# dselivanov/rsparse

Hardware: AMD Instinct MI355X
Metric: als_iterations_per_sec (higher is better)
Workload: dtype f32 (Gram products of rows > 512 / <= 32 non-zeros as 2 x fp16 / 3 x bf16 split terms of the fp32 operands, fp32 accumulate; everything else fp32); 1 GPU; WRMF implicit ALS, CG(3), synthetic 10000000x1000000, 500155883 nnz, rank 128, lambda 0.1; survey_config=3, feedback=implicit, n_items=1000000, nnz=500155883, rank=128, solver=conjugate_gradient, cg_steps=3, parallelism=rows sharded x1, factors replicated

## Files before the change

### rsparse_amd/build.py

```python
import subprocess
import sys
import time
from concurrent.futures import ThreadPoolExecutor
from pathlib import Path

PKG = Path(__file__).resolve().parent
CSRC = PKG / "csrc"
SRC = [CSRC / n for n in ("wrmf_kernels.hip", "wrmf_cgq.hip", "wrmf_cgp.hip", "wrmf_ne.hip", "wrmf_chol.hip", "wrmf_chol_wave.hip", "wrmf_chol_mf.hip", "wrmf_cg_mf.hip", "wrmf_chol_lr.hip",
                          "wrmf_topk.hip", "wrmf_topk_large.hip", "wrmf_similar.hip", "wrmf_metrics.hip", "wrmf_hits.hip", "wrmf_lists.hip", "wrmf_diversity.hip", "wrmf_mmr.hip", "wrmf_ranks.hip", "wrmf_score.hip", "wrmf_softals.hip", "wrmf_itemknn.hip", "wrmf_candidates.hip", "wrmf_sample.hip", "wrmf_sample_weighted.hip", "wrmf_split.hip", "wrmf_confidence.hip", "wrmf_events.hip", "wrmf_explain.hip", "wrmf_init.hip", "wrmf_ingest.hip", "wrmf_nnls.hip", "wrmf_bias.hip", "wrmf_lu.hip",
                          "wrmf_f64.hip", "wrmf_wide.hip", "wrmf_wide_cg.hip", "wrmf_ctx_kernels.hip", "wrmf_schedule.cpp", "wrmf_capi.cpp", "wrmf_f64_capi.cpp", "wrmf_capi_host.cpp", "wrmf_ctx.cpp")]
HEADERS = [CSRC / "wrmf_chol_mf.attrs.csv", CSRC / "wrmf_mf.h", CSRC / "wrmf_internal.h", CSRC / "wrmf_capi_common.h", CSRC / "wrmf_schedule.h", CSRC / "wrmf_device.h", CSRC / "wrmf_sample_team.h", CSRC / "wrmf_wave.h", CSRC / "wrmf_csr_rows.h", CSRC / "wrmf_ldlt.h", CSRC / "wrmf_f64.h", PKG.parent / "include" / "rsparse_wrmf_hip.h"]
DEPS = SRC + HEADERS
OUT = PKG / "lib" / "librsparse_wrmf_hip.so"
FLAGS = ["--offload-arch=gfx950", "-O3", "-std=c++17", "-fPIC"]


EXTRA_FLAGS = {n: ["-mllvm", "-forceattrs-csv-path=" + str(CSRC / "wrmf_chol_mf.attrs.csv"), "-fno-slp-vectorize"] for n in ("wrmf_chol_mf.hip", "wrmf_cg_mf.hip")}
AUDITED = {"wrmf_chol_mf.hip", "wrmf_cg_mf.hip"}
REG_LIMIT = {"wrmf_cg_mf.hip": 512}
NO_SPILL = {"wrmf_cgq.hip": ("14als_cgq_kernelILi128ELi24ELi4ELi4E",),
            "wrmf_cgp.hip": ("14als_cgp_kernelILb0ELb1ELi16ELb1E",),
            "wrmf_explain.hip": ("14explain_kernelIfLi128E",),
            "wrmf_sample.hip": ("13sample_kernelILi64E", "13sample_kernelILi256E"),
            "wrmf_sample_weighted.hip": ("22sample_weighted_kernelILi64E", "22sample_weighted_kernelILi256E"),
            "wrmf_hits.hip": ("18hit_metrics_kernelILb0E", "18hit_metrics_kernelILb1E"),
            "wrmf_lists.hip": ("19list_metrics_kernelILb0E", "19list_metrics_kernelILb1E"),
            "wrmf_diversity.hip": ("21list_diversity_kernelI", "21item_inv_norms_kernelI"),
            "wrmf_mmr.hip": ("10mmr_kernelI",),
            "wrmf_confidence.hip": ("conf_moments_kernel", "conf_moments_finish_kernel", "conf_table_kernel", "conf_apply_kernel"),
            "wrmf_events.hip": ("events_pack_kernel", "events_now_kernel", "events_heads_kernel", "events_reduce_kernel",
                                "events_long_chunks_kernel", "events_long_finish_kernel"),
            "wrmf_cg_mf.hip": ("rsparse_hip_als_cg_mf_implicit", "rsparse_hip_als_cg_mf_implicit_any"),
            "wrmf_softals.hip": ("softals_span_kernel", "softals_finish_kernel", "softals_empty_rows_kernel"),
            "wrmf_itemknn.hip": ("knn_scatter_kernel", "knn_mask_kernel", "knn_select_kernel"),
            "wrmf_split.hip": ("split_count_wave_kernel", "split_count_team_kernel", "split_write_wave_kernel", "split_write_team_kernel")}
RESOURCE_FLAG = "-Rpass-analysis=kernel-resource-usage"


def resource_violations(remarks, patterns, limit=256):
    import re
    rows, cur = [], None
    for line in remarks.splitlines():
        m = re.search(r"remark:\s+(.*?) \[-Rpass", line)
# ... 103 lines not shown
```

### rsparse_amd/csrc/wrmf_capi.cpp

```cpp
#include "../../include/rsparse_wrmf_hip.h"

#include <cxxabi.h>

#include <algorithm>
#include <cfloat>
#include <cmath>
#include <cstdlib>
#include <cstring>
#include <string>
#include <vector>

#include "wrmf_capi_common.h"

using namespace rsparse_hip;

struct rsparse_hip_csc {
  DevCSC d;
  int device = 0;
  std::vector<void*> owned;
};

namespace {
thread_local std::string g_err;
}
// ... 115 lines not shown
  if (int rc = upload(m, cut.segs, &L.segs)) return rc;
  if (int rc = upload(m, cut.split_rows, &L.split_rows)) return rc;
  return upload(m, cut.split_ptr, &L.split_ptr);
}
int upload_deal(rsparse_hip_csc& m, const NeDeal& deal, NeListSet& L) {
  L.wg = deal.wg();
  if (int rc = upload(m, deal.rows, &L.rows)) return rc;
  return upload(m, deal.ptr, &L.ptr);
}

int build_schedule(rsparse_hip_csc& m, const int32_t* host_col_ptrs) {
  DevCSC& d = m.d;
  int cus = 256;
  HIP_TRY(hipDeviceGetAttribute(&cus, hipDeviceAttributeMultiprocessorCount, m.device));
  d.q_cfg = cgq_default_cfg();
  SchedulePlan plan;
  if (!plan_schedule(host_col_ptrs, d.n_cols, cus, [](int len) { return cgq_bucket_of(len, cgq_default_cfg()); }, plan))
    return fail(RSPARSE_HIP_ERR_INVALID, "col_ptrs is not non-decreasing");
  d.max_len = plan.max_len; d.nnz_long = plan.nnz_long; d.n_empty = plan.n_empty;
  d.short_max = kTileNnz; d.n_long = plan.n_long;
  for (int b = 0; b < 7; b++) d.q_off[b] = plan.off[b];
  for (int b = 0; b < 6; b++) d.q_nnz[b] = plan.nnz[b];
  d.q_pair_first = plan.pair_first; d.q_team4_first = plan.team4_first;
  d.q_team4_wide_first = plan.team4_wide_first;
  d.q_gt32 = plan.gt32; d.q_gt48 = plan.gt48; d.q_lr_first = plan.lr_first; d.q_n_lr = plan.n_lr;
  d.q_n_chol_long = plan.n_chol_long; d.q_n_nec = plan.n_nec;
  int rc;
  if ((rc = upload(m, plan.order, &d.q_order))) return rc;
  if ((rc = upload(m, plan.stream_off, &d.q_stream_off))) return rc;
  if ((rc = upload_cut(m, plan.cut, d.q_ne))) return rc;
  d.q_ne1 = d.q_ne;
  if ((rc = upload_deal(m, plan.fine, d.q_ne))) return rc;
  if ((rc = upload_deal(m, plan.coarse, d.q_ne1))) return rc;
  if (plan.nec_is_ne) {
    d.q_nec = d.q_ne;
  } else {
    if ((rc = upload_cut(m, plan.cut_nec, d.q_nec))) return rc;
    if ((rc = upload_deal(m, plan.nec, d.q_nec))) return rc;
  }
  return RSPARSE_HIP_OK;
}

bool use_cgq(int rank, const void* X, const void* Y) {
  return rank % 4 == 0 && ((reinterpret_cast<uintptr_t>(X) | reinterpret_cast<uintptr_t>(Y)) & 15) == 0;
}

int check_common(int n_rows, int n_cols, const void* col_ptrs, const void* X, const void* Y, int rank) {
// ... 105 lines not shown
    a.rhs_vals = bias ? bias->rhs_vals : nullptr;
    a.loss_tgt = bias ? bias->loss_tgt : nullptr;
    a.rhs_init = bias ? bias->rhs_init : nullptr;
    a.loss_tgt_const = bias ? bias->tgt_const : 1.f;
    a.gbias = (solver == RSPARSE_SOLVER_CONJUGATE_GRADIENT && implicit && bias) ? bias->gbias : 0.f;
    const bool wave_cg = wide_cg_wave_supported(a, solver) && (d.q_order || d.max_len <= kWideCgMaxLen);
    hipError_t we = wave_cg ? launch_wide_cg_wave(a, implicit, kWideCgMaxLen, d.max_len > kWideCgMaxLen ? d.q_order : nullptr, 0, s)
                            : launch_als_wide(a, implicit, solver, g_ws.wide_m2, g_ws.wide_lu, s);
    if (we != hipSuccess) return hip_fail(we, wave_cg ? "launch_wide_cg_wave" : "launch_als_wide");
    if ((we = launch_sum_partials(g_ws.partials, wave_cg ? (size_t)grid_w : (size_t)grid, outw, s, g_ws.partials + g_ws.partial_slots())) != hipSuccess)
      return hip_fail(we, "launch_sum_partials");
    return RSPARSE_HIP_OK;
  }
  const bool cg = solver == RSPARSE_SOLVER_CONJUGATE_GRADIENT;
  const bool cgq = cg && use_cgq(rank, d_X, d_Y);
  QSchedule qs;
  qs.order = d.q_order;
  qs.cfg = d.q_cfg;
  qs.pair_first = d.q_pair_first;
  for (int b = 0; b < 7; b++) qs.off[b] = d.q_off[b];
  qs.team4_first = (implicit && bias && bias->gbias != 0.f) ? d.q_off[2] : d.q_team4_first;
  qs.team4_wide_first = (implicit && bias && bias->gbias != 0.f) ? d.q_off[2] : d.q_team4_wide_first;
  qs.pair_wide = cgp_wide_supported(rank, implicit, implicit && bias && bias->gbias != 0.f);
  qs.pair_quad = cgp_quad_supported(rank, implicit, implicit && bias && bias->gbias != 0.f);
  const bool cg_mf = cgq && implicit && !bias && cg_mf_supported(rank, implicit) && d.q_order && d.q_off[1] > d.q_n_nec;
  if (cg_mf) {
    qs.mf_rows = d.q_order + d.q_n_nec;
    qs.mf_n = d.q_off[1] - d.q_n_nec;
  }
  const bool chol_mf = chol_mf_supported(rank) && !cg && solver == RSPARSE_SOLVER_CHOLESKY && !bias && d.q_order && ne_supported(rank) &&
                       use_cgq(rank, d_X, d_Y) && d.q_lr_first > d.q_off[1];
  const int mf_first = d.q_off[1];
  const int n_mf = chol_mf ? d.q_lr_first - mf_first : 0;
  const bool nec_lists = padded_rank(rank) > 64 && d.q_nec.wg > 0 && !chol_mf;
  const bool ne_chol = !cg && solver == RSPARSE_SOLVER_CHOLESKY && !bias && (nec_lists || d.q_ne.wg > 0 || chol_mf) &&
                       ne_supported(rank) && use_cgq(rank, d_X, d_Y);
  qs.ne = (cg_mf || (ne_chol && nec_lists)) ? d.q_nec : ((implicit && padded_rank(rank) == 128) ? d.q_ne : d.q_ne1);
  const size_t chol_base = chol2_loss_slots(d.n_cols);
  const size_t slots = cgq ? cgq_loss_slots(qs, rank, implicit) : (cg ? cg_loss_slots(d.n_cols, d.n_long)
                                   : (solver == RSPARSE_SOLVER_NNLS ? chol_loss_slots(d.n_cols)
                                      : chol_base + (ne_chol ? (size_t)(qs.ne.entries + qs.ne.nsplit) : 0) +
                                            (size_t)(chol_mf ? chol_mf_loss_slots(n_mf, implicit) : 0) + (size_t)kLuGrid));
  if ((rc = g_ws.ensure_partials(slots))) return rc;
  double* out = d_loss_rows_out ? d_loss_rows_out : g_ws.scalars;
  if (d.n_cols == 0) {
    HIP_TRY(hipMemsetAsync(out, 0, sizeof(double), s));
// ... 1307 lines not shown
```

### rsparse_amd/csrc/wrmf_cgq.hip

```cpp
#include <algorithm>

#include "wrmf_internal.h"
#include "wrmf_device.h"

namespace rsparse_hip {
namespace {

using namespace dev;

constexpr int kGvFirstMinCapq = 16;
constexpr int kStreamPrefixQ = 4;
constexpr int kIdxPrefetchMaxWpr = 2;

constexpr int kMaxSavedSweeps = 4;

template <int KP>
struct QG {
  static constexpr int RPN = KP / 16;
  static constexpr int VW = RPN >= 4 ? 4 : RPN;
  static constexpr int NV = RPN / VW;
  __device__ static __forceinline__ int elem(int i, int r) { return (r / VW) * (16 * VW) + i * VW + (r % VW); }
};

template <int VW>
struct Piece;
template <>
struct Piece<4> { using type = float4; };
template <>
struct Piece<2> { using type = float2; };

__device__ __forceinline__ float groups_reduce_scatter4(const float a0, const float a1, const float a2, const float a3) {
  const auto s01 = __builtin_amdgcn_permlane16_swap(__float_as_uint(a0), __float_as_uint(a1), false, false);
  const float c = __uint_as_float(s01[0]) + __uint_as_float(s01[1]);
  const auto s23 = __builtin_amdgcn_permlane16_swap(__float_as_uint(a2), __float_as_uint(a3), false, false);
  const float d = __uint_as_float(s23[0]) + __uint_as_float(s23[1]);
  const auto t = __builtin_amdgcn_permlane32_swap(__float_as_uint(c), __float_as_uint(d), false, false);
  return __uint_as_float(t[0]) + __uint_as_float(t[1]);
}
template <int KP, int CAPQ, int WAVES, int WPR, int STREAM, bool IMPLICIT, int DMF = 0>
struct QSmem {
  static constexpr size_t gram_floats = (IMPLICIT && DMF != 1) ? (size_t)KP * KP : 0;
  static constexpr size_t vec_floats = IMPLICIT ? (size_t)WAVES * KP : 0;
  static constexpr size_t red_floats = WPR > 1 ? (size_t)2 * WAVES * KP + 2 * WAVES : 0;
  static constexpr bool cv_lds = !STREAM && CAPQ * (KP / 16) > 128;
  static constexpr bool wideq = !STREAM && CAPQ * (KP / 16) > 160;
  static constexpr size_t tsv_floats = (STREAM && !IMPLICIT) ? 0 : (size_t)WAVES * (cv_lds ? 3 : 2) * CAPQ * 4;
  static constexpr size_t pre_floats = STREAM ? (size_t)WAVES * kStreamPrefixQ * 4 * KP : 0;
  static constexpr int dmf_ps = KP + 8, dmf_os = KP + 4;
  static constexpr size_t dmf_floats = DMF ? (size_t)WAVES * dmf_ps + (size_t)WAVES * dmf_os : 0;
  static constexpr size_t pfx_floats =
      (!STREAM && WPR > kIdxPrefetchMaxWpr && (CAPQ == 16 || CAPQ == 20 || CAPQ == 24)) ? (size_t)WAVES * 2 * CAPQ * 4 : 0;
  static constexpr size_t wl_floats = cv_lds ? (size_t)WAVES * 2 : 0;
  static constexpr size_t xs_floats = cv_lds ? (size_t)WAVES * KP : 0;
  static constexpr size_t bytes =
      (gram_floats + vec_floats + red_floats + tsv_floats + pre_floats + dmf_floats + pfx_floats + wl_floats + xs_floats) * 4 + 16;
};

template <int KP, int CAPQ, int WAVES, int WPR, int STREAM, bool IMPLICIT, int DMF = 0, bool GB = false, bool KFULL = false>
__global__ __launch_bounds__(WAVES * 64, 2) void als_cgq_kernel(AlsArgs a, const int32_t* __restrict__ rows, int n_rows,
                                                             int rows_per_team, size_t loss_slot0) {
  using G_ = QG<KP>;
  constexpr int RPN = G_::RPN, VW = G_::VW, NV = G_::NV, CAP = CAPQ * 4, TEAMS = WAVES / WPR;
  using piece_t = typename Piece<VW>::type;
  using SM = QSmem<KP, CAPQ, WAVES, WPR, STREAM, IMPLICIT, DMF>;
  static_assert(WAVES % WPR == 0, "teams must tile the workgroup");
  constexpr bool GRS = RPN == 8 && VW == 4;
  auto groups_all_reduce8 = [](float(&a8)[RPN]) {
    if constexpr (RPN == 8) {
      const float r0 = groups_reduce_scatter4(a8[0], a8[1], a8[2], a8[3]);
      const float r1 = groups_reduce_scatter4(a8[4], a8[5], a8[6], a8[7]);
      float g0[4], g1[4];
      rows_to_all<4>(r0, g0);
      rows_to_all<4>(r1, g1);
#pragma unroll
      for (int e = 0; e < 4; e++) a8[e] = g0[e], a8[4 + e] = g1[e];
    }
  };
  static_assert(!DMF || (IMPLICIT && KP == 128 && WAVES == 4 && WPR == 1 && STREAM == 0), "DMF geometry");
  static_assert(DMF != 1 || CAPQ == 8, "register-resident G terms: only the 8-quad kernel has the 64 registers");
  static_assert(!GB || IMPLICIT, "the global bias of explicit feedback is removed from the data (R/model_WRMF.R:278-282)");
  const float gbias = GB ? a.gbias : 0.f, ltgt = GB ? a.loss_tgt_const : 1.f;
  extern __shared__ __attribute__((aligned(16))) char smem[];
  float* sG = reinterpret_cast<float*>(smem);
  float* sVec = sG + SM::gram_floats;
  float* sRed = sVec + SM::vec_floats;
  float* sRedL = sRed + (WPR > 1 ? 2 * WAVES * KP : 0);
  float* sTsv = sVec + SM::vec_floats + SM::red_floats;
  float* sPre = sTsv + SM::tsv_floats;
  float* sPfx = sPre + SM::pre_floats;
  _Float16* sPh = reinterpret_cast<_Float16*>(sPre + SM::pre_floats);
  _Float16* sPl = sPh + WAVES * SM::dmf_ps;
  float* sOut = reinterpret_cast<float*>(sPl + WAVES * SM::dmf_ps);

  const int tid = threadIdx.x, lane = tid & 63, wv = rfl(tid >> 6);
  const int g = lane >> 4, i = lane & 15;
  const int team = wv / WPR, tw = wv % WPR;
  const int k = KFULL ? KP : a.k;
  if constexpr (IMPLICIT && DMF == 0) {
    constexpr int GU = (KP * KP) % (8 * WAVES * 64) == 0 ? 8 : ((KP * KP) % (2 * WAVES * 64) == 0 ? 2 : 1);
    static_assert((KP * KP) % (GU * WAVES * 64) == 0, "the Gramian copy walks whole batches");
    for (int e0 = tid; e0 < KP * KP; e0 += GU * WAVES * 64) {
      float gv[GU];
#pragma unroll
      for (int u = 0; u < GU; u++) {
        const int e = e0 + u * WAVES * 64, r = e / KP, c = e % KP;
        gv[u] = a.XtX[(size_t)min(r, k - 1) * k + min(c, k - 1)];
      }
#pragma unroll
      for (int u = 0; u < GU; u++) {
        const int e = e0 + u * WAVES * 64, r = e / KP, c = e % KP;
        sG[e] = (r < k && c < k) ? gv[u] : 0.f;
      }
// ... 76 lines not shown
  const int team_global = blockIdx.x * TEAMS + team;
  const int total_teams = gridDim.x * TEAMS;

  auto row_index = [&](int itn) { return team_global + itn * total_teams; };
  int row_c = 0, p1_c = 0, p2_c = 0, row_n = 0;
  if (rows_per_team > 0 && row_index(0) < n_rows) {
    row_c = rows[row_index(0)];
    p1_c = a.col_ptrs[row_c];
    p2_c = a.col_ptrs[row_c + 1];
  }
  if (rows_per_team > 1 && row_index(1) < n_rows) row_n = rows[row_index(1)];
  for (int it = 0; it < rows_per_team; ++it) {
    const int ri = row_index(it);
    const bool have = ri < n_rows;
    if (WPR == 1 && !DMF && !have) break;
    const int row = have ? rfl(row_c) : 0;
    const int p1 = have ? rfl(p1_c) : 0;
    const int p2 = have ? rfl(p2_c) : 0;
    constexpr bool META_LATE = WIDEQ && !KFULL;
#define RSP_ADVANCE_META()                                                      \
    {                                                                           \
      int p1_n = 0, p2_n = 0, row_nn = 0;                                       \
      if (it + 1 < rows_per_team && row_index(it + 1) < n_rows) {               \
        p1_n = a.col_ptrs[row_n];                                               \
        p2_n = a.col_ptrs[row_n + 1];                                           \
      }                                                                         \
      if (it + 2 < rows_per_team && row_index(it + 2) < n_rows) row_nn = rows[row_index(it + 2)]; \
      row_c = row_n;                                                            \
      p1_c = p1_n;                                                              \
      p2_c = p2_n;                                                              \
      row_n = row_nn;                                                           \
    }
    if constexpr (!META_LATE) RSP_ADVANCE_META()
    const int cnt = p2 - p1;
    float* yrow = a.Y + (size_t)row * k;
    if (!GB && WPR == 1 && cnt <= 0) {
      if (!DMF || have)
        for (int e = lane; e < k; e += 64) yrow[e] = 0.f;
      if constexpr (!DMF) continue;
    }
    constexpr int PQ = STREAM ? kStreamPrefixQ : 0, PCAP = PQ * 4, PTEAM = PCAP * WPR;
    const int pre = STREAM ? min(cnt, PTEAM) : 0;
    const int pw = STREAM ? max(0, min(PCAP, pre - tw * PCAP)) : 0;
    const int nchunks = (cnt - pre + CAP - 1) / CAP;
    constexpr bool resident = STREAM == 0;
    const float lam_use =
        IMPLICIT ? 0.f : (float)(a.lambda_loss * (a.dynamic_lambda ? (double)(float)cnt : 1.0));

// ... 256 lines not shown
      float lacc = 0.f;
      float vinv = 0.f;
      if constexpr (DMF) {
        if (mode != 2) {
          float vmax = 0.f;
#pragma unroll
          for (int rr = 0; rr < RPN; rr++) vmax = fmaxf(vmax, fabsf(v[rr]));
          vmax = row16_max(vmax);
          const int ve = fp16_scale_exp(vmax);
          const float vs = __uint_as_float((unsigned)ve << 23);
          vinv = __uint_as_float((unsigned)(254 - ve) << 23) * (mode == 0 ? -1.f : 1.f);
          if (g < NV) {
            float w4[VW];
#pragma unroll
            for (int c = 0; c < VW; c++) w4[c] = (g == 0 ? v[c] : v[VW + c]) * vs;
            unsigned h0, l0, h1, l1;
            split_f16(w4[0], w4[1], h0, l0);
            split_f16(w4[2], w4[3], h1, l1);
            const int off = wv * SM::dmf_ps + g * 16 * VW + i * VW;
            *reinterpret_cast<uint2*>(sPh + off) = make_uint2(h0, h1);
            *reinterpret_cast<uint2*>(sPl + off) = make_uint2(l0, l1);
          }
          __syncthreads();
          f32x4 d0[2], d1[2];
#pragma unroll
          for (int t = 0; t < 2; t++) d0[t] = d1[t] = f32x4{0.f, 0.f, 0.f, 0.f};
          const int nb = (lane & 3) * SM::dmf_ps + 8 * (lane >> 4);
#pragma unroll
          for (int ks = 0; ks < 4; ks++) {
            const f16x8 bh = *reinterpret_cast<const f16x8*>(sPh + nb + 32 * ks);
            const f16x8 bl = *reinterpret_cast<const f16x8*>(sPl + nb + 32 * ks);
#pragma unroll
            for (int t = 0; t < 2; t++) {
              f16x8 ah, al;
              if constexpr (DMF == 1) {
                ah = gAh[t][ks];
                al = gAl[t][ks];
              } else {
                ah = *reinterpret_cast<const f16x8*>(sGf + ((t * 4 + ks) * 2 + 0) * 1024 + lane * 16);
                al = *reinterpret_cast<const f16x8*>(sGf + ((t * 4 + ks) * 2 + 1) * 1024 + lane * 16);
              }
              d0[t] = __builtin_amdgcn_mfma_f32_16x16x32_f16(ah, bh, d0[t], 0, 0, 0);
              d1[t] = __builtin_amdgcn_mfma_f32_16x16x32_f16(ah, bl, d1[t], 0, 0, 0);
              d1[t] = __builtin_amdgcn_mfma_f32_16x16x32_f16(al, bh, d1[t], 0, 0, 0);
            }
          }
          if ((lane & 15) < 4) {
#pragma unroll
            for (int t = 0; t < 2; t++) {
              const f32x4 d = (d0[t] + d1[t]) * ginv;
              *reinterpret_cast<f32x4*>(sOut + (lane & 15) * SM::dmf_os + 32 * wv + 16 * t + 4 * (lane >> 4)) = d;
            }
          }
        }
      }
      if (live) {
        if constexpr (IMPLICIT && !DMF) {
          if (mode != 2) {
            wave_sync();
            if (g == 0) {
#pragma unroll
              for (int b = 0; b < NV; b++) {
                piece_t pc;
                float* pf = reinterpret_cast<float*>(&pc);
#pragma unroll
                for (int c = 0; c < VW; c++) pf[c] = v[b * VW + c];
                *reinterpret_cast<piece_t*>(vec + b * 16 * VW + i * VW) = pc;
              }
            }
            wave_sync();
          }
        }
        auto dense_part = [&]() {
          if (IMPLICIT && !DMF && mode != 2) {
            const float sign = mode == 0 ? -1.f : 1.f;
// ... 330 lines not shown
    }
  }
  if (lane == 0) a.loss_partials[loss_slot0 + (size_t)blockIdx.x * WAVES + wv] = CVLDS ? *wl_lds : wloss;
}

struct BucketDef { int waves, wpr, capq, stream, max_len; };
constexpr int kNB = 6;
constexpr int kNCfg = 2;
constexpr BucketDef kBuckets[kNCfg][kNB] = {
    {{8, 8, 16, 1, 0x7fffffff}, {8, 8, 16, 0, 512}, {4, 4, 16, 0, 256}, {4, 2, 16, 0, 128}, {4, 1, 16, 0, 64}, {4, 1, 8, 0, 32}},
    {{8, 8, 16, 1, 0x7fffffff}, {4, 4, 32, 0, 512}, {4, 2, 32, 0, 256}, {4, 1, 32, 0, 128}, {4, 1, 16, 0, 64}, {4, 1, 8, 0, 32}},
};
constexpr int cfg_of_kp(int KP) { return KP == 64 ? 1 : 0; }
constexpr int kTeam4Waves = 4, kTeam4Capq = 20;
static_assert(kTeam4Max == kTeam4Waves * kTeam4Capq * 4, "wrmf_internal.h's split and the kernel's capacity");
constexpr int kTeam4WideCapq = 24;
static_assert(kTeam4WideMax == kTeam4Waves * kTeam4WideCapq * 4, "wrmf_schedule.h's split and the wide kernel's capacity");
static_assert(kTeam4Max < kTeam4WideMax && kTeam4WideMax < 512, "the 4-wave launches take bucket 1's rows from its short end");
static_assert(QSmem<128, kTeam4WideCapq, kTeam4Waves, kTeam4Waves, 0, true>::bytes <= 80 * 1024, "the wide team kernel's LDS");
constexpr bool team4_split(int KP, bool GB) { return KP == 128 && !GB; }
int team4_first(const QSchedule& q) { return std::min(std::max(q.team4_first, q.off[1]), q.off[2]); }
int team4_wide_first(const QSchedule& q) { return std::min(std::max(q.team4_wide_first, q.off[1]), team4_first(q)); }

template <int KP, int WAVES, int CAPQ, int WPR, int STREAM, bool IMPLICIT, bool GB, int DMF = 0, bool KFULL = false>
hipError_t launch_bucket(const AlsArgs& a, const int32_t* rows, int n_rows, int grid, size_t slot0, hipStream_t s,
                         hipEvent_t* ev_slot) {
  if (n_rows <= 0) return hipSuccess;
  constexpr bool kDmfGeometry = IMPLICIT && KP == 128 && WAVES == 4 && WPR == 1 && (CAPQ == 8 || CAPQ == 16) && STREAM == 0;
  if constexpr (kDmfGeometry && !DMF) {
    return launch_bucket<KP, WAVES, CAPQ, WPR, STREAM, IMPLICIT, GB, CAPQ == 8 ? 1 : 2>(a, rows, n_rows, grid, slot0, s, ev_slot);
  } else {
    if constexpr (!KFULL && STREAM == 0 && !(DMF == 1 && !GB)) {
      if (a.k == KP)
        return launch_bucket<KP, WAVES, CAPQ, WPR, STREAM, IMPLICIT, GB, DMF, true>(a, rows, n_rows, grid, slot0, s, ev_slot);
    }
    constexpr int TEAMS = WAVES / WPR;
    auto kern = als_cgq_kernel<KP, CAPQ, WAVES, WPR, STREAM, IMPLICIT, DMF, GB, KFULL>;
    const size_t lds = QSmem<KP, CAPQ, WAVES, WPR, STREAM, IMPLICIT, DMF>::bytes;
    hipError_t err = hipFuncSetAttribute(reinterpret_cast<const void*>(kern),
                                         hipFuncAttributeMaxDynamicSharedMemorySize, (int)lds);
    if (err != hipSuccess) return err;
    const int total_teams = grid * TEAMS;
    const int rpt = (n_rows + total_teams - 1) / total_teams;
    prof_note(ev_slot, reinterpret_cast<const void*>(kern));
    hipLaunchKernelGGL(kern, dim3(grid), dim3(WAVES * 64), lds, s, a, rows, n_rows, rpt, slot0);
    return hipGetLastError();
// ... 15 lines not shown
    if ((err = hipEventCreateWithFlags(&fork0, hipEventDisableTiming)) != hipSuccess) return err;
    for (int b = 0; b < kNB; b++) {
      if ((err = hipStreamCreateWithFlags(&st[b], hipStreamNonBlocking)) != hipSuccess) return err;
      if ((err = hipEventCreateWithFlags(&done[b], hipEventDisableTiming)) != hipSuccess) return err;
    }
    return hipSuccess;
  }
};
thread_local BucketStreams g_bs;

int g_launch_mode = 2;
int concurrent_buckets() { return g_launch_mode; }

size_t bucket_slots(const QSchedule& q, int b, int k, bool implicit) {
  const int cfg = cfg_of_kp(padded_rank(k));
  const BucketDef d = kBuckets[cfg][b];
  if (d.wpr <= 0) return 0;
  if (d.stream && ne_supported(k)) return (size_t)(q.ne.entries + q.ne.nsplit) + (size_t)(q.mf_n > 0 ? cg_mf_loss_slots(q.mf_n) : 0);
  const int rows = q.off[b + 1] - q.off[b];
  if (b == 1 && padded_rank(k) == 128) {
    const int wide = team4_wide_first(q), split = team4_first(q);
    return (size_t)cgq_bucket_grid(wide - q.off[b], b, cfg) * d.waves + (size_t)cgq_team4_wide_grid(split - wide) * kTeam4Waves +
           (size_t)cgq_team4_grid(q.off[b + 1] - split) * kTeam4Waves;
  }
  if (b == kNB - 1 && rows > 0 && cgp_supported(k, implicit)) {
    const int split = std::min(std::max(q.pair_first, q.off[b]), q.off[b + 1]);
    const size_t main = q.pair_wide ? (size_t)cgp_loss_slots(split - q.off[b], cgp_rows_per_wave(kCgpWide))
                                    : (size_t)cgq_bucket_grid(split - q.off[b], b, cfg) * d.waves;
    return main + (size_t)cgp_loss_slots(q.off[b + 1] - split, cgp_rows_per_wave(q.pair_quad ? kCgpQuad : kCgpPair));
  }
  return (size_t)cgq_bucket_grid(rows, b, cfg) * d.waves;
}

template <int KP, int CFG, bool IMPLICIT, bool GB>
hipError_t launch_all(const AlsArgs& a, const QSchedule& q, hipStream_t s, hipEvent_t* ev) {
  hipError_t err;
  size_t slot = 0;
  const int cmode = ev ? 0 : concurrent_buckets();
  const bool overlap = cmode != 0;
  bool forked = false;
  if (overlap) {
    if ((err = g_bs.ensure()) != hipSuccess) return err;
  }
#define RSP_BUCKET(B)                                                                                       \
  {                                                                                                         \
    constexpr BucketDef D = kBuckets[CFG][B];                                                               \
// ... 37 lines not shown
              if ((err = hipStreamWaitEvent(s, g_bs.done[B], 0)) != hipSuccess) return err;                 \
            }                                                                                               \
          }                                                                                                 \
        } else if constexpr (D.stream && KP > 32) {        \
          return hipErrorInvalidValue;                                                                      \
        } else if constexpr (B == 1 && team4_split(KP, GB)) {                                              \
           \
           \
          const int first = q.off[B], wide = team4_wide_first(q), split = team4_first(q);                   \
          const int n_main = wide - first, n_w4 = split - wide, n_t4 = q.off[B + 1] - split;                \
          const int g_main = cgq_bucket_grid(n_main, B, CFG), g_w4 = cgq_team4_wide_grid(n_w4);             \
          if ((err = launch_bucket<KP, D.waves, D.capq, D.wpr, D.stream, IMPLICIT, GB>(a, q.order + first, n_main, g_main, slot, \
                                                                                  bs, ev ? ev + B : nullptr)) != hipSuccess) \
            return err;                                                                                     \
          if ((err = launch_bucket<KP, kTeam4Waves, kTeam4WideCapq, kTeam4Waves, 0, IMPLICIT, GB>(          \
                   a, q.order + wide, n_w4, g_w4, slot + (size_t)g_main * D.waves, bs,                      \
                   n_main > 0 ? nullptr : (ev ? ev + B : nullptr))) != hipSuccess)                          \
            return err;                                                                                     \
          if ((err = launch_bucket<KP, kTeam4Waves, kTeam4Capq, kTeam4Waves, 0, IMPLICIT, GB>(              \
                   a, q.order + split, n_t4, cgq_team4_grid(n_t4),                                          \
                   slot + (size_t)g_main * D.waves + (size_t)g_w4 * kTeam4Waves, bs,                        \
                   n_main + n_w4 > 0 ? nullptr : (ev ? ev + B : nullptr))) != hipSuccess)                   \
            return err;                                                                                     \
        } else if (B == kNB - 1 && cgp_supported(a.k, IMPLICIT)) {                    \
           \
                  \
          const int first = q.off[B], split = std::min(std::max(q.pair_first, first), q.off[B + 1]);         \
          const int n_main = split - first, n_pair = q.off[B + 1] - split;                                   \
          size_t main_slots;                                                                                \
          if (q.pair_wide) {                                                                                \
            if ((err = launch_als_cgp(a, q.order + first, n_main, kCgpWide, slot, bs, ev ? ev + B : nullptr)) != hipSuccess) \
              return err;                                                                                   \
            main_slots = (size_t)cgp_loss_slots(n_main, cgp_rows_per_wave(kCgpWide));                       \
          } else {                                                                                          \
            const int g_main = cgq_bucket_grid(n_main, B, CFG);                                             \
            if ((err = launch_bucket<KP, D.waves, D.capq, D.wpr, D.stream, IMPLICIT, GB>(a, q.order + first, n_main, g_main, slot, \
                                                                                    bs, ev ? ev + B : nullptr)) != hipSuccess) \
              return err;                                                                                   \
            main_slots = (size_t)g_main * D.waves;                                                          \
          }                                                                                                 \
          if ((err = launch_als_cgp(a, q.order + split, n_pair, q.pair_quad ? kCgpQuad : kCgpPair, slot + main_slots, bs, \
                                    n_main > 0 ? nullptr : (ev ? ev + B : nullptr))) != hipSuccess)           \
            return err;                                                                                     \
        } else if ((err = launch_bucket<KP, D.waves, D.capq, D.wpr, D.stream, IMPLICIT, GB>(a, q.order + q.off[B], n, grid, slot, \
                                                                                bs, ev ? ev + B : nullptr)) != hipSuccess) \
          return err;                                                                                       \
// ... 40 lines not shown
int cgq_bucket_grid(int n_rows, int b, int cfg) {
  const BucketDef d = kBuckets[cfg][b];
  if (n_rows <= 0 || d.wpr <= 0) return 0;
  const int base = d.stream ? 16 : (d.wpr == 1 ? 64 : (d.wpr == 2 ? 64 : 32));
  return team_grid(n_rows, d.waves / d.wpr, base);
}

int cgq_team4_grid(int n_rows) { return n_rows <= 0 ? 0 : team_grid(n_rows, 1, 32); }
int cgq_team4_wide_grid(int n_rows) { return cgq_team4_grid(n_rows); }

int cgq_bucket_of(int len, int cfg) {
  int best = 0;
  for (int b = 0; b < kNB; b++)
    if (kBuckets[cfg][b].wpr > 0 && len <= kBuckets[cfg][b].max_len) best = b;
  return best;
}

size_t cgq_loss_slots(const QSchedule& q, int k, bool implicit) {
  size_t n = 0;
  for (int b = 0; b < kNB; b++) n += bucket_slots(q, b, k, implicit);
  return n;
}

int cgq_default_cfg() { return 0; }
void cgq_set_launch_mode(int mode) { g_launch_mode = mode; }

hipError_t launch_als_cgq(const AlsArgs& a, const QSchedule& q, bool implicit, hipStream_t s, hipEvent_t* ev) {
  const int KP = padded_rank(a.k);
#define RSP_DISPATCH(KPV)                                                                                   \
  if (KP == KPV) {                                                                                          \
    if (implicit && a.gbias != 0.f) return launch_all<KPV, cfg_of_kp(KPV), true, true>(a, q, s, ev);        \
    return implicit ? launch_all<KPV, cfg_of_kp(KPV), true, false>(a, q, s, ev)                             \
                    : launch_all<KPV, cfg_of_kp(KPV), false, false>(a, q, s, ev);                           \
  }
  RSP_DISPATCH(32)
  RSP_DISPATCH(64)
  RSP_DISPATCH(128)
#undef RSP_DISPATCH
  return hipErrorInvalidValue;
}

}
```

### rsparse_amd/csrc/wrmf_internal.h

```cpp
#pragma once
#include <hip/hip_runtime.h>
#include <cstdint>
#include <string>

#include "wrmf_schedule.h"

namespace rsparse_hip {

constexpr float kCgTol = 1e-10f;
constexpr double kCgTolD = 1e-10;
constexpr int kScdMaxIter = 10000;
constexpr float kScdTol = 1e-4f;
constexpr double kScdTolD = 1e-4;
constexpr float kNnlsEps = 1e-16f;
constexpr double kNnlsEpsD = 1e-16;

struct NeListSet {
  const int32_t* rows = nullptr;
  const int32_t* ptr = nullptr;
  int wg = 0;
  int entries = 0;
  const int32_t* segs = nullptr;
  int nseg = 0;
  const int32_t* split_rows = nullptr;
  const int32_t* split_ptr = nullptr;
  int nsplit = 0;
};

struct DevCSC {
  int n_rows = 0;
  int n_cols = 0;
  int64_t nnz = 0;
  const int32_t* col_ptrs = nullptr;
  const int32_t* row_idx = nullptr;
  const float* vals = nullptr;
  int n_long = 0;
  int short_max = 0;
  int max_len = 0;
  const int32_t* q_order = nullptr;
  int q_off[7] = {0, 0, 0, 0, 0, 0, 0};
  int q_cfg = 0;
  int q_pair_first = 0;
  int q_team4_first = 0;
  int q_team4_wide_first = 0;
  int64_t q_nnz[6] = {0, 0, 0, 0, 0, 0};
  const int64_t* q_stream_off = nullptr;
  int q_n_chol_long = 0;
  int q_gt32 = 0;
  int q_gt48 = 0;
  int q_lr_first = 0, q_n_lr = 0;
  NeListSet q_ne;
  NeListSet q_ne1;
  int q_n_nec = 0;
  NeListSet q_nec;
  int64_t nnz_long = 0;
  int n_empty = 0;
  mutable bool vals_frozen = false;
  mutable bool vstats_valid = false;
  mutable unsigned* vstats = nullptr;
  mutable hipStream_t vstats_stream = nullptr;
};

struct AlsArgs {
  const int32_t* col_ptrs;
  const int32_t* row_idx;
  const float* vals;
  const float* X;
// ... 32 lines not shown
  int lr_n_gt48;
  float* nnls_lhs;
  const int32_t* nnls_order;
  int lrx;
  unsigned* lr_flags;
  float* lr_M;
  const int32_t* ne_segs;
  float* ne_seg_scratch;
  int* ne_seg_flags;
  int ne_chol;
  int ne_chol_min;
  const unsigned* ne_stats;
  const float* mf_XtX;
  const unsigned* wave_stats;
};

struct QSchedule {
  const int32_t* order;
  int off[7];
  int pair_first;
  int team4_first;
  int team4_wide_first;
  bool pair_wide;
  bool pair_quad = false;
  int cfg;
  NeListSet ne;
  const int32_t* mf_rows = nullptr;
  int mf_n = 0;
};
int cgq_default_cfg();
void cgq_set_launch_mode(int mode);
int cgq_num_buckets();
int cgq_bucket_wpr(int cfg, int b);
int cgq_bucket_capq(int cfg, int b);
int cgq_bucket_waves(int cfg, int b);
int cgq_bucket_stream(int cfg, int b);
int cgq_bucket_grid(int n_rows, int bucket, int cfg);
int cgq_team4_grid(int n_rows);
int cgq_team4_wide_grid(int n_rows);
int cgq_bucket_of(int len, int cfg);
size_t cgq_loss_slots(const QSchedule& q, int k, bool implicit);
bool cgp_supported(int k, bool implicit);
bool cgp_wide_supported(int k, bool implicit, bool gbias);
bool cgp_quad_supported(int k, bool implicit, bool gbias);
enum CgpForm { kCgpPair = 0, kCgpWide = 1, kCgpQuad = 2 };
inline int cgp_rows_per_wave(CgpForm form) { return form == kCgpQuad ? 4 : 2; }
hipError_t launch_als_cgp(const AlsArgs& a, const int32_t* rows, int n_rows, CgpForm form, size_t loss_slot0, hipStream_t s,
                          hipEvent_t* ev_slot);
bool ne_supported(int k);
constexpr int kNeMinLen = 512;
constexpr int kNeSegFloats = 4 * (11 * 16 * 64 + 128 + 2);
hipError_t launch_ne_stats(const float* X, int64_t nx, const float* vals, int64_t nnz, unsigned* stats, hipStream_t s,
                           const float* absmax_hint = nullptr, const unsigned* cached_vstats = nullptr,
                           unsigned* save_vstats = nullptr);
hipError_t launch_als_ne(const AlsArgs& a, const QSchedule& q, bool implicit, double* row_loss, hipStream_t s,
                         hipEvent_t* ev_slot = nullptr);
hipError_t launch_gb_row_terms(const AlsArgs& a, const int32_t* rows, int n, float* out, int32_t* slot_of_row, hipStream_t s);
hipError_t launch_als_cgq(const AlsArgs& a, const QSchedule& q, bool implicit, hipStream_t s, hipEvent_t* ev = nullptr);

constexpr int kWavesPerWG = 4;
constexpr int kRowsPerWGShort = 64;
constexpr int kRowsPerWGLong = 8;
// ... 292 lines not shown
```

### rsparse_amd/csrc/wrmf_schedule.cpp

```cpp
#include "wrmf_schedule.h"

#include <algorithm>
#include <functional>
#include <queue>
#include <utility>

namespace rsparse_hip {

namespace {
int ne_slots(int cus) { return 2 * std::max(cus, 1); }
}

int cgp_grid(int n_rows, int rows_per_wave) {
  if (n_rows <= 0) return 0;
  const long sets = ((long)n_rows + rows_per_wave - 1) / rows_per_wave;
  long per_wave = 32;
  const long spread = 4L * 512;
  if (sets < spread * per_wave) per_wave = (sets + spread - 1) / spread;
  if (per_wave < 1) per_wave = 1;
  return (int)((sets + 4 * per_wave - 1) / (4 * per_wave));
}
int cgp_visits(int n_rows, int rows_per_wave) {
  const long grid = cgp_grid(n_rows, rows_per_wave);
  if (grid <= 0) return 0;
  const long sets = ((long)n_rows + rows_per_wave - 1) / rows_per_wave;
  return (int)((sets + grid * 4 - 1) / (grid * 4));
}
int64_t cgp_loss_slots(int n_rows, int rows_per_wave) { return (int64_t)cgp_grid(n_rows, rows_per_wave) * 4; }

NeCut ne_cut(const int32_t* order, const int32_t* col_ptrs, int n_prefix, int64_t fixed, int cus) {
  NeCut c;
  if (n_prefix <= 0) return c;
  auto len_of = [&](int r) { return (int64_t)(col_ptrs[order[r] + 1] - col_ptrs[order[r]]); };
  auto steps_of = [](int64_t len) { return (len + 15) / 16; };
  const int n_slots = ne_slots(cus);
  int64_t total = 0;
  for (int r = 0; r < n_prefix; r++) total += steps_of(len_of(r)) + fixed;
  const int64_t share = std::max<int64_t>(1, total / n_slots);
  c.items.reserve((size_t)n_prefix + 64);
  int n_seg = 0;
  for (int r = 0; r < n_prefix; r++) {
    const int64_t len = len_of(r);
    const int64_t st = steps_of(len);
    int parts = 1;
    if (n_slots >= 8 && 2 * (st + fixed) > share)
      parts = (int)std::min<int64_t>(std::min<int64_t>(kNeMaxSeg, st / 64), (4 * st + share - 1) / share);
    if (parts < 2 || n_seg + parts > kNeMaxSegTotal) {
      c.items.push_back({st + fixed, order[r]});
      continue;
    }
    const int64_t per = (st + parts - 1) / parts;
// ... 46 lines not shown
  for (int i = 0; i < n; i++) {
    const int len = col_ptrs[i + 1] - col_ptrs[i];
    if (len < 0) return false;
    max_len = std::max(max_len, len);
  }
  out.max_len = max_len;
  if (n <= 0) {
    out.nec_is_ne = true;
    return true;
  }
  std::vector<int64_t> start((size_t)max_len + 2, 0);
  for (int i = 0; i < n; i++) start[(size_t)(max_len - (col_ptrs[i + 1] - col_ptrs[i])) + 1]++;
  int cnt_b[6] = {0, 0, 0, 0, 0, 0};
  for (int len = max_len; len >= 0; len--) {
    const int cnt = (int)start[(size_t)(max_len - len) + 1];
    if (!cnt) continue;
    if (len > kTileNnz) { out.n_long += cnt; out.nnz_long += (int64_t)len * cnt; }
    if (len == 0) out.n_empty += cnt;
    if (len > kCholLongLen) out.n_chol_long += cnt;
    if (len > kCgMfMax) out.n_nec += cnt;
    if (len > 16) out.pair_first += cnt;
    if (len > kTeam4Max) out.team4_first += cnt;
    if (len > kTeam4WideMax) out.team4_wide_first += cnt;
    if (len > 32) out.gt32 += cnt;
    if (len > 48) out.gt48 += cnt;
    if (len > kCholLrMax) out.lr_first += cnt;
    else if (len >= 1) out.n_lr += cnt;
    const int b = bucket_of(len);
    cnt_b[b] += cnt;
    out.nnz[b] += (int64_t)len * cnt;
  }
  for (int b = 0; b < 6; b++) out.off[b + 1] = out.off[b] + cnt_b[b];
  for (size_t b = 1; b < start.size(); b++) start[b] += start[b - 1];
  out.order.resize((size_t)n);
  for (int i = 0; i < n; i++) out.order[(size_t)start[(size_t)(max_len - (col_ptrs[i + 1] - col_ptrs[i]))]++] = i;
  const int n_stream = out.off[1];
  if (n_stream > 0) {
    out.stream_off.assign((size_t)n_stream + 1, 0);
    for (int r = 0; r < n_stream; r++) {
      const int row = out.order[(size_t)r];
      out.stream_off[(size_t)r + 1] = out.stream_off[(size_t)r] + (col_ptrs[row + 1] - col_ptrs[row]);
    }
    out.cut = ne_cut(out.order.data(), col_ptrs, n_stream, 12, cus);
    out.fine = ne_deal(out.cut, n_stream, cus, true);
    out.coarse = ne_deal(out.cut, n_stream, cus, false);
  }
// ... 10 lines not shown
```

### rsparse_amd/csrc/wrmf_schedule.h

```cpp
#pragma once
#include <cstdint>
#include <vector>

namespace rsparse_hip {

constexpr int kTileNnz = 32;
constexpr int kTeam4Max = 320;
constexpr int kTeam4WideMax = 384;
constexpr int kCholLrMax = 64;
constexpr int kCholLongLen = 4096;
constexpr int kCgMfMax = 16384;
constexpr int kNeMaxSeg = 16;
constexpr int kNeMaxSegTotal = 1024;

int cgp_grid(int n_rows, int rows_per_wave = 2);
int cgp_visits(int n_rows, int rows_per_wave = 2);
int64_t cgp_loss_slots(int n_rows, int rows_per_wave = 2);

struct NeCut {
  struct Item { int64_t cost; int32_t entry; };
  std::vector<Item> items;
  std::vector<int32_t> segs;
  std::vector<int32_t> split_rows;
  std::vector<int32_t> split_ptr;
  int nseg() const { return (int)(segs.size() / 6); }
};
struct NeDeal {
  std::vector<int32_t> rows, ptr;
  int wg() const { return ptr.empty() ? 0 : (int)ptr.size() - 1; }
};

NeCut ne_cut(const int32_t* order, const int32_t* col_ptrs, int n_prefix, int64_t fixed, int cus);
NeDeal ne_deal(const NeCut& cut, int n_prefix, int cus, bool fine);

struct SchedulePlan {
  int max_len = 0;
  int n_long = 0;
  int64_t nnz_long = 0;
  int n_empty = 0;
  std::vector<int32_t> order;
  int off[7] = {0, 0, 0, 0, 0, 0, 0};
  int64_t nnz[6] = {0, 0, 0, 0, 0, 0};
  int pair_first = 0;
  int team4_first = 0;
  int team4_wide_first = 0;
  int gt32 = 0, gt48 = 0;
  int lr_first = 0, n_lr = 0;
  int n_chol_long = 0;
  int n_nec = 0;
  std::vector<int64_t> stream_off;
  NeCut cut, cut_nec;
  NeDeal fine, coarse, nec;
  bool nec_is_ne = false;
};

bool plan_schedule(const int32_t* col_ptrs, int n_cols, int cus, int (*bucket_of)(int len), SchedulePlan& out);

}
```

Baseline: 8.711 iterations/s.

## Split bucket 3 at 96 nnz and route short rows to a one-wave-per-row MFMA CG kernel

Adds a schedule split inside bucket 3 that sends rows with at most 96 non-zeros to a new one-wave-per-row CG kernel (CAPQ 24, DMF 2). That kernel computes its Gram product with split-fp16 MFMA, prefetches indices into LDS and reads col_ptrs through the constant address space. The aim is to stop spending a multi-wave team on mid-length rows and so improve occupancy and load balance. In exchange it adds another kernel launch, more loss-slot bookkeeping and a new LDS layout, and it changes where sPfx sits in the DMF layout.

```diff
diff --git a/rsparse_amd/build.py b/rsparse_amd/build.py
--- a/rsparse_amd/build.py
+++ b/rsparse_amd/build.py
@@ -18,7 +18,7 @@
 EXTRA_FLAGS = {n: ["-mllvm", "-forceattrs-csv-path=" + str(CSRC / "wrmf_chol_mf.attrs.csv"), "-fno-slp-vectorize"] for n in ("wrmf_chol_mf.hip", "wrmf_cg_mf.hip")}
 AUDITED = {"wrmf_chol_mf.hip", "wrmf_cg_mf.hip"}
 REG_LIMIT = {"wrmf_cg_mf.hip": 512}
-NO_SPILL = {"wrmf_cgq.hip": ("14als_cgq_kernelILi128ELi24ELi4ELi4E",),
+NO_SPILL = {"wrmf_cgq.hip": ("14als_cgq_kernelILi128ELi24ELi4ELi",),
             "wrmf_cgp.hip": ("14als_cgp_kernelILb0ELb1ELi16ELb1E",),
             "wrmf_explain.hip": ("14explain_kernelIfLi128E",),
             "wrmf_sample.hip": ("13sample_kernelILi64E", "13sample_kernelILi256E"),
diff --git a/rsparse_amd/csrc/wrmf_capi.cpp b/rsparse_amd/csrc/wrmf_capi.cpp
--- a/rsparse_amd/csrc/wrmf_capi.cpp
+++ b/rsparse_amd/csrc/wrmf_capi.cpp
@@ -161,7 +161,7 @@
   for (int b = 0; b < 7; b++) d.q_off[b] = plan.off[b];
   for (int b = 0; b < 6; b++) d.q_nnz[b] = plan.nnz[b];
   d.q_pair_first = plan.pair_first; d.q_team4_first = plan.team4_first;
-  d.q_team4_wide_first = plan.team4_wide_first;
+  d.q_team4_wide_first = plan.team4_wide_first; d.q_wave_wide_first = plan.wave_wide_first;
   d.q_gt32 = plan.gt32; d.q_gt48 = plan.gt48; d.q_lr_first = plan.lr_first; d.q_n_lr = plan.n_lr;
   d.q_n_chol_long = plan.n_chol_long; d.q_n_nec = plan.n_nec;
   int rc;
@@ -313,6 +313,7 @@
   qs.team4_first = (implicit && bias && bias->gbias != 0.f) ? d.q_off[2] : d.q_team4_first;
   qs.team4_wide_first = (implicit && bias && bias->gbias != 0.f) ? d.q_off[2] : d.q_team4_wide_first;
   qs.pair_wide = cgp_wide_supported(rank, implicit, implicit && bias && bias->gbias != 0.f);
+  qs.wave_wide_first = (!bias && cgq_wave_wide_supported(rank, implicit, false)) ? d.q_wave_wide_first : d.q_off[4];
   qs.pair_quad = cgp_quad_supported(rank, implicit, implicit && bias && bias->gbias != 0.f);
   const bool cg_mf = cgq && implicit && !bias && cg_mf_supported(rank, implicit) && d.q_order && d.q_off[1] > d.q_n_nec;
   if (cg_mf) {
diff --git a/rsparse_amd/csrc/wrmf_cgq.hip b/rsparse_amd/csrc/wrmf_cgq.hip
--- a/rsparse_amd/csrc/wrmf_cgq.hip
+++ b/rsparse_amd/csrc/wrmf_cgq.hip
@@ -36,6 +36,10 @@
   const float d = __uint_as_float(s23[0]) + __uint_as_float(s23[1]);
   const auto t = __builtin_amdgcn_permlane32_swap(__float_as_uint(c), __float_as_uint(d), false, false);
   return __uint_as_float(t[0]) + __uint_as_float(t[1]);
+}
+__device__ __forceinline__ int const_i32(const int32_t* p, const int idx) {
+  using cint = const __attribute__((address_space(4))) int32_t;
+  return reinterpret_cast<cint*>(reinterpret_cast<uintptr_t>(p))[idx];
 }
 template <int KP, int CAPQ, int WAVES, int WPR, int STREAM, bool IMPLICIT, int DMF = 0>
 struct QSmem {
@@ -48,8 +52,9 @@
   static constexpr size_t pre_floats = STREAM ? (size_t)WAVES * kStreamPrefixQ * 4 * KP : 0;
   static constexpr int dmf_ps = KP + 8, dmf_os = KP + 4;
   static constexpr size_t dmf_floats = DMF ? (size_t)WAVES * dmf_ps + (size_t)WAVES * dmf_os : 0;
+  static constexpr bool wave_wide = DMF == 2 && CAPQ == 24;
   static constexpr size_t pfx_floats =
-      (!STREAM && WPR > kIdxPrefetchMaxWpr && (CAPQ == 16 || CAPQ == 20 || CAPQ == 24)) ? (size_t)WAVES * 2 * CAPQ * 4 : 0;
+      (!STREAM && (WPR > kIdxPrefetchMaxWpr || wave_wide) && (CAPQ == 16 || CAPQ == 20 || CAPQ == 24)) ? (size_t)WAVES * 2 * CAPQ * 4 : 0;
   static constexpr size_t wl_floats = cv_lds ? (size_t)WAVES * 2 : 0;
   static constexpr size_t xs_floats = cv_lds ? (size_t)WAVES * KP : 0;
   static constexpr size_t bytes =
@@ -87,7 +92,7 @@
   float* sRedL = sRed + (WPR > 1 ? 2 * WAVES * KP : 0);
   float* sTsv = sVec + SM::vec_floats + SM::red_floats;
   float* sPre = sTsv + SM::tsv_floats;
-  float* sPfx = sPre + SM::pre_floats;
+  float* sPfx = sPre + SM::pre_floats + SM::dmf_floats;
   _Float16* sPh = reinterpret_cast<_Float16*>(sPre + SM::pre_floats);
   _Float16* sPl = sPh + WAVES * SM::dmf_ps;
   float* sOut = reinterpret_cast<float*>(sPl + WAVES * SM::dmf_ps);
@@ -210,8 +215,16 @@
     {                                                                           \
       int p1_n = 0, p2_n = 0, row_nn = 0;                                       \
       if (it + 1 < rows_per_team && row_index(it + 1) < n_rows) {               \
-        p1_n = a.col_ptrs[row_n];                                               \
-        p2_n = a.col_ptrs[row_n + 1];                                           \
+         \
+         \
+                        \
+        if constexpr (SM::wave_wide) {                                          \
+          p1_n = const_i32(a.col_ptrs, row_n);                                  \
+          p2_n = const_i32(a.col_ptrs, row_n + 1);                              \
+        } else {                                                                \
+          p1_n = a.col_ptrs[row_n];                                             \
+          p2_n = a.col_ptrs[row_n + 1];                                         \
+        }                                                                       \
       }                                                                         \
       if (it + 2 < rows_per_team && row_index(it + 2) < n_rows) row_nn = rows[row_index(it + 2)]; \
       row_c = row_n;                                                            \
@@ -514,6 +527,30 @@
             *reinterpret_cast<uint2*>(sPl + off) = make_uint2(l0, l1);
           }
           __syncthreads();
+          if constexpr (SM::wave_wide) {
+            const int ln = opaque_lane<true>(lane);
+            const int nbw = (ln & 3) * SM::dmf_ps + 8 * (ln >> 4);
+            const char* gf = reinterpret_cast<const char*>(sG) + (size_t)wv * 16 * 1024 + ln * 16;
+#pragma unroll
+            for (int t = 0; t < 2; t++) {
+              f32x4 e0 = {0.f, 0.f, 0.f, 0.f}, e1 = {0.f, 0.f, 0.f, 0.f};
+#pragma unroll
+              for (int ks = 0; ks < 4; ks++) {
+                const f16x8 bh = *reinterpret_cast<const f16x8*>(sPh + nbw + 32 * ks);
+                const f16x8 bl = *reinterpret_cast<const f16x8*>(sPl + nbw + 32 * ks);
+                const f16x8 ah = *reinterpret_cast<const f16x8*>(gf + ((t * 4 + ks) * 2 + 0) * 1024);
+                const f16x8 al = *reinterpret_cast<const f16x8*>(gf + ((t * 4 + ks) * 2 + 1) * 1024);
+                e0 = __builtin_amdgcn_mfma_f32_16x16x32_f16(ah, bh, e0, 0, 0, 0);
+                e1 = __builtin_amdgcn_mfma_f32_16x16x32_f16(ah, bl, e1, 0, 0, 0);
+                e1 = __builtin_amdgcn_mfma_f32_16x16x32_f16(al, bh, e1, 0, 0, 0);
+                __builtin_amdgcn_sched_barrier(0);
+              }
+              if ((ln & 15) < 4) {
+                const f32x4 d = (e0 + e1) * ginv;
+                *reinterpret_cast<f32x4*>(sOut + (ln & 15) * SM::dmf_os + 32 * wv + 16 * t + 4 * (ln >> 4)) = d;
+              }
+            }
+          } else {
           f32x4 d0[2], d1[2];
 #pragma unroll
           for (int t = 0; t < 2; t++) d0[t] = d1[t] = f32x4{0.f, 0.f, 0.f, 0.f};
@@ -543,6 +580,7 @@
               const f32x4 d = (d0[t] + d1[t]) * ginv;
               *reinterpret_cast<f32x4*>(sOut + (lane & 15) * SM::dmf_os + 32 * wv + 16 * t + 4 * (lane >> 4)) = d;
             }
+          }
           }
         }
       }
@@ -919,6 +957,25 @@
 int team4_first(const QSchedule& q) { return std::min(std::max(q.team4_first, q.off[1]), q.off[2]); }
 int team4_wide_first(const QSchedule& q) { return std::min(std::max(q.team4_wide_first, q.off[1]), team4_first(q)); }
 
+constexpr int kWaveWideCapq = 24;
+static_assert(kWaveWideMax == kWaveWideCapq * 4, "wrmf_schedule.h's split and the one-wave wide kernel's capacity");
+static_assert(kWaveWideMax > kBuckets[0][4].max_len && kWaveWideMax < kBuckets[0][3].max_len, "the split lies inside bucket 3");
+static_assert(QSmem<128, kWaveWideCapq, 4, 1, 0, true, 2>::bytes <= 80 * 1024, "the one-wave wide kernel's LDS");
+constexpr bool wave_wide_split(int KP, bool IMPLICIT, bool GB) { return KP == 128 && IMPLICIT && !GB; }
+int wave_wide_first(const QSchedule& q) { return std::min(std::max(q.wave_wide_first, q.off[3]), q.off[4]); }
+
+hipError_t launch_wave_wide(const AlsArgs& a, const int32_t* rows, int n_rows, size_t slot0, hipStream_t s, hipEvent_t* ev_slot) {
+  if (n_rows <= 0) return hipSuccess;
+  if (a.k != 128) return hipErrorInvalidValue;
+  auto kern = als_cgq_kernel<128, kWaveWideCapq, 4, 1, 0, true, 2, false, true>;
+  const size_t lds = QSmem<128, kWaveWideCapq, 4, 1, 0, true, 2>::bytes;
+  hipError_t err = hipFuncSetAttribute(reinterpret_cast<const void*>(kern), hipFuncAttributeMaxDynamicSharedMemorySize, (int)lds);
+  if (err != hipSuccess) return err;
+  prof_note(ev_slot, reinterpret_cast<const void*>(kern));
+  hipLaunchKernelGGL(kern, dim3(cgq_wave_wide_grid(n_rows)), dim3(4 * 64), lds, s, a, rows, n_rows, cgq_wave_wide_visits(n_rows), slot0);
+  return hipGetLastError();
+}
+
 template <int KP, int WAVES, int CAPQ, int WPR, int STREAM, bool IMPLICIT, bool GB, int DMF = 0, bool KFULL = false>
 hipError_t launch_bucket(const AlsArgs& a, const int32_t* rows, int n_rows, int grid, size_t slot0, hipStream_t s,
                          hipEvent_t* ev_slot) {
@@ -980,6 +1037,10 @@
     const int wide = team4_wide_first(q), split = team4_first(q);
     return (size_t)cgq_bucket_grid(wide - q.off[b], b, cfg) * d.waves + (size_t)cgq_team4_wide_grid(split - wide) * kTeam4Waves +
            (size_t)cgq_team4_grid(q.off[b + 1] - split) * kTeam4Waves;
+  }
+  if (b == 3 && padded_rank(k) == 128) {
+    const int split = wave_wide_first(q);
+    return (size_t)cgq_bucket_grid(split - q.off[b], b, cfg) * d.waves + (size_t)cgq_wave_wide_loss_slots(q.off[b + 1] - split);
   }
   if (b == kNB - 1 && rows > 0 && cgp_supported(k, implicit)) {
     const int split = std::min(std::max(q.pair_first, q.off[b]), q.off[b + 1]);
@@ -1063,6 +1124,18 @@
                    slot + (size_t)g_main * D.waves + (size_t)g_w4 * kTeam4Waves, bs,                        \
                    n_main + n_w4 > 0 ? nullptr : (ev ? ev + B : nullptr))) != hipSuccess)                   \
             return err;                                                                                     \
+        } else if constexpr (B == 3 && wave_wide_split(KP, IMPLICIT, GB)) {                                 \
+           \
+                  \
+          const int first = q.off[B], split = wave_wide_first(q);                                           \
+          const int n_main = split - first, n_ww = q.off[B + 1] - split;                                    \
+          const int g_main = cgq_bucket_grid(n_main, B, CFG);                                               \
+          if ((err = launch_bucket<KP, D.waves, D.capq, D.wpr, D.stream, IMPLICIT, GB>(a, q.order + first, n_main, g_main, slot, \
+                                                                                  bs, ev ? ev + B : nullptr)) != hipSuccess) \
+            return err;                                                                                     \
+          if ((err = launch_wave_wide(a, q.order + split, n_ww, slot + (size_t)g_main * D.waves, bs,        \
+                                      n_main > 0 ? nullptr : (ev ? ev + B : nullptr))) != hipSuccess)       \
+            return err;                                                                                     \
         } else if (B == kNB - 1 && cgp_supported(a.k, IMPLICIT)) {                    \
            \
                   \
@@ -1149,6 +1222,8 @@
   return n;
 }
 
+bool cgq_wave_wide_supported(int k, bool implicit, bool gbias) { return implicit && k == 128 && !gbias; }
+
 int cgq_default_cfg() { return 0; }
 void cgq_set_launch_mode(int mode) { g_launch_mode = mode; }
 
diff --git a/rsparse_amd/csrc/wrmf_internal.h b/rsparse_amd/csrc/wrmf_internal.h
--- a/rsparse_amd/csrc/wrmf_internal.h
+++ b/rsparse_amd/csrc/wrmf_internal.h
@@ -43,6 +43,7 @@
   int q_pair_first = 0;
   int q_team4_first = 0;
   int q_team4_wide_first = 0;
+  int q_wave_wide_first = 0;
   int64_t q_nnz[6] = {0, 0, 0, 0, 0, 0};
   const int64_t* q_stream_off = nullptr;
   int q_n_chol_long = 0;
@@ -121,6 +122,7 @@
   int team4_first;
   int team4_wide_first;
   bool pair_wide;
+  int wave_wide_first = 0x7fffffff;
   bool pair_quad = false;
   int cfg;
   NeListSet ne;
@@ -137,6 +139,7 @@
 int cgq_bucket_grid(int n_rows, int bucket, int cfg);
 int cgq_team4_grid(int n_rows);
 int cgq_team4_wide_grid(int n_rows);
+bool cgq_wave_wide_supported(int k, bool implicit, bool gbias);
 int cgq_bucket_of(int len, int cfg);
 size_t cgq_loss_slots(const QSchedule& q, int k, bool implicit);
 bool cgp_supported(int k, bool implicit);
diff --git a/rsparse_amd/csrc/wrmf_schedule.cpp b/rsparse_amd/csrc/wrmf_schedule.cpp
--- a/rsparse_amd/csrc/wrmf_schedule.cpp
+++ b/rsparse_amd/csrc/wrmf_schedule.cpp
@@ -27,6 +27,21 @@
   return (int)((sets + grid * 4 - 1) / (grid * 4));
 }
 int64_t cgp_loss_slots(int n_rows, int rows_per_wave) { return (int64_t)cgp_grid(n_rows, rows_per_wave) * 4; }
+
+int cgq_wave_wide_grid(int n_rows) {
+  if (n_rows <= 0) return 0;
+  long per_wave = 64;
+  const long spread = 4L * 512;
+  if (n_rows < spread * per_wave) per_wave = (n_rows + spread - 1) / spread;
+  if (per_wave < 1) per_wave = 1;
+  return (int)((n_rows + 4 * per_wave - 1) / (4 * per_wave));
+}
+int cgq_wave_wide_visits(int n_rows) {
+  const long grid = cgq_wave_wide_grid(n_rows);
+  if (grid <= 0) return 0;
+  return (int)((n_rows + grid * 4 - 1) / (grid * 4));
+}
+int64_t cgq_wave_wide_loss_slots(int n_rows) { return (int64_t)cgq_wave_wide_grid(n_rows) * 4; }
 
 NeCut ne_cut(const int32_t* order, const int32_t* col_ptrs, int n_prefix, int64_t fixed, int cus) {
   NeCut c;
@@ -119,6 +134,7 @@
     if (len > 16) out.pair_first += cnt;
     if (len > kTeam4Max) out.team4_first += cnt;
     if (len > kTeam4WideMax) out.team4_wide_first += cnt;
+    if (len > kWaveWideMax) out.wave_wide_first += cnt;
     if (len > 32) out.gt32 += cnt;
     if (len > 48) out.gt48 += cnt;
     if (len > kCholLrMax) out.lr_first += cnt;
diff --git a/rsparse_amd/csrc/wrmf_schedule.h b/rsparse_amd/csrc/wrmf_schedule.h
--- a/rsparse_amd/csrc/wrmf_schedule.h
+++ b/rsparse_amd/csrc/wrmf_schedule.h
@@ -7,6 +7,7 @@
 constexpr int kTileNnz = 32;
 constexpr int kTeam4Max = 320;
 constexpr int kTeam4WideMax = 384;
+constexpr int kWaveWideMax = 96;
 constexpr int kCholLrMax = 64;
 constexpr int kCholLongLen = 4096;
 constexpr int kCgMfMax = 16384;
@@ -16,6 +17,10 @@
 int cgp_grid(int n_rows, int rows_per_wave = 2);
 int cgp_visits(int n_rows, int rows_per_wave = 2);
 int64_t cgp_loss_slots(int n_rows, int rows_per_wave = 2);
+
+int cgq_wave_wide_grid(int n_rows);
+int cgq_wave_wide_visits(int n_rows);
+int64_t cgq_wave_wide_loss_slots(int n_rows);
 
 struct NeCut {
   struct Item { int64_t cost; int32_t entry; };
@@ -44,6 +49,7 @@
   int pair_first = 0;
   int team4_first = 0;
   int team4_wide_first = 0;
+  int wave_wide_first = 0;
   int gt32 = 0, gt48 = 0;
   int lr_first = 0, n_lr = 0;
   int n_chol_long = 0;
```

After: 8.768 iterations/s (median of 6 runs). Within noise of the previous version (+0.7%).
